# isunLt/U2MKD

Hardware: AMD Instinct MI355X
Metric: LiDAR points/sec/node fwd+bwd (teacher+student+KD), 1/2/4/8 MI355X (higher is better)
Workload: dtype f32 (fp32 products emulated on the 16-bit matrix pipe: f16x2 forward / input gradient, bf16x3 weight gradient; fp32 accumulate)

## Files before the change

include/u2mkd_hip.h:

```cpp
#ifndef U2MKD_HIP_H
#define U2MKD_HIP_H

#include <stddef.h>
#include <stdint.h>

#ifdef __cplusplus
extern "C" {
#endif

typedef void *u2mkd_stream_t;

int u2mkd_version(void);
const char *u2mkd_last_error(void);
int u2mkd_stream_wait_stream(u2mkd_stream_t waiter, u2mkd_stream_t signaler);
void *u2mkd_mailbox_alloc(size_t bytes);
int u2mkd_mailbox_free(void *p);
int u2mkd_mailbox_post(const void *const *srcs, uint32_t is64, int32_t n, int64_t *slot, int64_t seq, u2mkd_stream_t s);

int u2mkd_hash(const int32_t *coords , int64_t n, int64_t *out , u2mkd_stream_t s);
int u2mkd_kernel_hash(const int32_t *coords , const int32_t *offsets , int64_t n,
                      int32_t k, int64_t *out , u2mkd_stream_t s);

size_t u2mkd_hash_table_bytes(int64_t n_refs);
int u2mkd_hash_table_build(const int64_t *refs, int64_t n_refs, void *table, u2mkd_stream_t s);
// ... 358 lines not shown
                                          const int32_t *sort_idx, const int32_t *wstart, const int32_t *wlen,
                                          const int32_t *qc, const float *radial, const float *tq, const float *tk,
                                          const float *tv, int32_t L, int32_t qgl, float split_a, int32_t qc_span,
                                          int64_t n, int32_t h, int32_t hdim, float *delta ,
                                          void *workspace, size_t workspace_bytes, float *dq, float *dk, float *dv,
                                          int64_t ld_grad, float *dtq, float *dtk, float *dtv, u2mkd_stream_t s);
#include "u2mkd_hip_sptr_rows16.h"

int u2mkd_sptr_table_reduce(const void *workspace, int64_t n, int32_t h, int32_t L, float split_a, float *dtq, float *dtk,
                            float *dtv, u2mkd_stream_t s);

int u2mkd_sptr_quant_coords_shifted(const float *xyz , const int32_t *sort_idx , int64_t n, const float *lo,
                                    float wx, float wy, float wz, float shx, float shy, float shz, float qx, float qy,
                                    float qz, int32_t *qc , float *radial , u2mkd_stream_t s);

int u2mkd_sptr_plain_forward_strided(const float *q, const float *k, const float *v, int64_t ld_qkv, float q_scale,
                                     const int32_t *sort_idx, const int32_t *wstart, const int32_t *wlen, int64_t n,
                                     int32_t h, int32_t hdim, float *out, int64_t ld_out, float *lse, u2mkd_stream_t s);
int u2mkd_sptr_plain_backward_strided(const float *q, const float *k, const float *v, int64_t ld_qkv, float q_scale,
                                      const float *out, const float *dout, int64_t ld_out, const float *lse,
                                      const int32_t *sort_idx, const int32_t *wstart, const int32_t *wlen, int64_t n,
                                      int32_t h, int32_t hdim, float *delta , float *dq, float *dk,
                                      float *dv, int64_t ld_grad, u2mkd_stream_t s);

int u2mkd_sptr_precompute_all(int32_t N, int32_t n, uint32_t n_max, const int32_t *counts, const int32_t *offsets,
                              const int32_t *sq_offsets, int32_t *index_0_offsets, int32_t *index_1_offsets,
                              int32_t *index_0, int32_t *index_1, u2mkd_stream_t s);
int u2mkd_sptr_attention_step1_forward(int32_t N_q, int32_t N_k, int32_t M, int32_t h, int32_t hdim, uint32_t n_max,
                                       const float *q, const float *k, const int32_t *index0, const int32_t *index1,
                                       float *attn, u2mkd_stream_t s);
int u2mkd_sptr_attention_step1_backward(int32_t N, int32_t M, int32_t h, int32_t hdim, uint32_t n_max,
                                        const float *grad_out, const int32_t *index0, const int32_t *index0_offsets,
                                        const int32_t *index1, const int32_t *index1_offsets, const float *q,
                                        const float *k, float *grad_q, float *grad_k, u2mkd_stream_t s);
int u2mkd_sptr_attention_step2_forward(int32_t N, int32_t M, int32_t h, int32_t hdim, int32_t n_max, const float *attn,
                                       const float *v, const int32_t *index0_offsets, const int32_t *index1,
                                       float *output, u2mkd_stream_t s);
int u2mkd_sptr_attention_step2_backward(int32_t N, int32_t M, int32_t h, int32_t hdim, int32_t n_max,
                                        const float *grad_out, const int32_t *index0, const int32_t *index0_offsets,
                                        const int32_t *index1, const int32_t *index1_offsets, const float *attn,
                                        const float *v, float *grad_attn, float *grad_v, u2mkd_stream_t s);
int u2mkd_sptr_dot_prod_with_idx_forward(int32_t N, int32_t M, int32_t h, int32_t hdim, int32_t n_max, int32_t L,
                                         const float *q, const int32_t *index_q, const int32_t *index_q_offsets,
                                         const float *k, const int32_t *index_k, const float *table_q,
                                         const float *table_k, const int32_t *rel_idx, float *output,
                                         u2mkd_stream_t s);
int u2mkd_sptr_dot_prod_with_idx_all_forward(int32_t N, int32_t M, int32_t h, int32_t hdim, int32_t n_max, int32_t L,
                                             const float *q, const int32_t *index_q, const int32_t *index_q_offsets,
                                             const float *k, const int32_t *index_k, const float *table_q,
                                             const float *table_k, const int32_t *rel_idx, float *output,
                                             u2mkd_stream_t s);
int u2mkd_sptr_dot_prod_with_idx_backward(int32_t N, int32_t M, int32_t h, int32_t hdim, int32_t n_max, int32_t L,
                                          const float *grad_out, const float *q, const int32_t *index_q_offsets,
                                          const float *k, const int32_t *index_k_offsets, const int32_t *index_k,
                                          const float *table_q, const float *table_k, const int32_t *rel_idx,
                                          float *grad_q, float *grad_k, float *grad_table_q, float *grad_table_k,
                                          u2mkd_stream_t s);
int u2mkd_sptr_attention_step2_with_rel_pos_value_forward(int32_t N, int32_t M, int32_t h, int32_t hdim, int32_t n_max,
                                                          const float *attn, const float *v,
                                                          const int32_t *index0_offsets, const int32_t *index1,
                                                          const float *table, const int32_t *rel_idx, float *output,
                                                          u2mkd_stream_t s);
int u2mkd_sptr_attention_step2_with_rel_pos_value_backward(int32_t N, int32_t M, int32_t h, int32_t hdim, int32_t L,
                                                           int32_t n_max, const float *grad_out, const int32_t *index0,
                                                           const int32_t *index0_offsets, const int32_t *index1,
                                                           const int32_t *index1_offsets, const float *attn,
                                                           const float *v, const float *table, const int32_t *rel_idx,
                                                           float *grad_attn, float *grad_v, float *grad_table,
                                                           u2mkd_stream_t s);

size_t u2mkd_bn2d_workspace_bytes(int64_t b, int32_t c, int64_t hw);
int u2mkd_bn2d_train_forward(const float *x, const float *res, int64_t b, int32_t c, int64_t hw, const float *gamma,
                             const float *beta, float eps, float momentum, int32_t relu, float *running_mean,
                             float *running_var, int64_t *num_batches_tracked, void *workspace,
                             float *mean , float *invstd , float *y, u2mkd_stream_t s);
int u2mkd_bn2d_eval_forward(const float *x, const float *res, int64_t b, int32_t c, int64_t hw, const float *gamma,
                            const float *beta, float eps, int32_t relu, const float *running_mean,
                            const float *running_var, float *y, u2mkd_stream_t s);
int u2mkd_bn2d_backward(const float *dy, const float *x, const float *res, int64_t b, int32_t c, int64_t hw,
                        const float *mean, const float *invstd, const float *gamma, const float *beta, int32_t relu,
                        int32_t batch_stats, void *workspace, float *dgamma, float *dbeta, float *dx,
                        float *dres , u2mkd_stream_t s);

int u2mkd_bn2d_local_stats(const float *x, int64_t b, int32_t c, int64_t hw, void *workspace, float *stats ,
                           u2mkd_stream_t s);
int u2mkd_bn2d_apply(const float *x, const float *res, int64_t b, int32_t c, int64_t hw, const float *mean,
                     const float *invstd, const float *gamma, const float *beta, int32_t relu, float *y, u2mkd_stream_t s);
int u2mkd_bn2d_backward_local(const float *dy, const float *x, const float *res, int64_t b, int32_t c, int64_t hw,
                              const float *mean, const float *invstd, const float *gamma, const float *beta, int32_t relu,
                              void *workspace, float *sums , float *keep ,
                              u2mkd_stream_t s);
int u2mkd_bn2d_backward_apply(const float *dy, const float *x, const float *res, int64_t b, int32_t c, int64_t hw,
                              const float *total_n , const float *mean, const float *invstd, const float *gamma,
                              const float *beta, int32_t relu, const float *sums , float *dx,
                              float *dres , u2mkd_stream_t s);

size_t u2mkd_sptr_tiles_workspace_bytes(int64_t n, int32_t h);
int u2mkd_sptr_attention_forward_tiles(const float *q, const float *k, const float *v, int64_t ld_qkv, float q_scale,
                                       const int32_t *sort_idx, const int32_t *wstart, const int32_t *wlen, const int32_t *qc,
                                       const float *radial, const float *tq, const float *tk, const float *tv, int32_t L,
                                       int32_t qgl, float split_a, int64_t n, int32_t h, int32_t hdim, float *out, int64_t ld_out,
                                       float *lse, void *workspace, size_t workspace_bytes, u2mkd_stream_t s);

int32_t u2mkd_sgd_chunk_elements(void);
int u2mkd_sgd_batch(const int64_t *jobs, int32_t n_jobs, int64_t total_chunks, float lr, float momentum, float weight_decay,
                    int32_t nesterov, int32_t contract, u2mkd_stream_t s);
int u2mkd_grads_unscale_check(const int64_t *jobs, int32_t n_jobs, int64_t total_chunks, const float *inv_scale, float *found_inf,
                              u2mkd_stream_t s);
int u2mkd_sgd_batch_amp(const int64_t *jobs, int32_t n_jobs, int64_t total_chunks, float lr, float momentum, float weight_decay,
                        int32_t nesterov, int32_t contract, const float *grad_scale, const float *found_inf, u2mkd_stream_t s);
int u2mkd_adam_batch(const int64_t *jobs, int32_t n_jobs, int64_t total_chunks, const float *scalars, float decay, float weight_decay,
                     int32_t decoupled, float w1, float beta2, float w2, float eps, int32_t form, u2mkd_stream_t s);
int u2mkd_adam_batch_amp(const int64_t *jobs, int32_t n_jobs, int64_t total_chunks, const float *scalars, int32_t window, float decay,
                         float weight_decay, int32_t decoupled, float w1, float beta2, float w2, float eps, int32_t form,
                         const int32_t *count_in, int32_t *count_out, int32_t count_known, const float *grad_scale,
                         const float *found_inf, u2mkd_stream_t s);
int u2mkd_debug_adam_stage(int32_t stage, int32_t form, const float *a, const float *b, const float *c, float scalar, float *out,
                           int64_t n, u2mkd_stream_t s);

size_t u2mkd_prep_scan_workspace_bytes(int64_t n);
int32_t u2mkd_prep_key_bits(int32_t axis);
int u2mkd_prep_sweep_compact(const float *sweep, int64_t m, void *workspace, int32_t *pos, u2mkd_stream_t s);
int u2mkd_prep_points(const float *key, const int64_t *labels, int64_t nk, const float *sweep, int64_t m, const void *workspace,
                      const int32_t *pos, const int32_t *kseg, const int32_t *mseg, const int32_t *sseg, int32_t n_sweeps,
                      const double *tm, int32_t nb, const double *par, const int32_t *flip, int32_t train, int32_t f32mode,
                      double voxel_size, int64_t ignore_label, float *feats, int32_t *vox, int64_t *labels_full, uint8_t *kf,
                      int32_t *mn, int32_t *off, u2mkd_stream_t s);
int u2mkd_prep_project(const float *key, int64_t nk, const int32_t *kseg, int32_t nb, int32_t ncam, const double *cam, float *pc,
                       uint8_t *masks, uint8_t *pt_with_img, u2mkd_stream_t s);
int u2mkd_prep_voxel_keys(const int32_t *vox, const int32_t *mn, const int32_t *off, int32_t nb, int64_t cap, int64_t *keys,
                          int32_t *err, u2mkd_stream_t s);
int u2mkd_prep_voxel_sets(const int64_t *skeys, const int64_t *perm, int64_t cap, void *workspace, int32_t *rank,
                          const int32_t *off, int32_t nb, const float *feats, const int32_t *vox, const int32_t *mn,
                          const int64_t *labels, const uint8_t *kf, const uint8_t *pt_with_img, const uint8_t *masks,
                          const float *pc, int32_t ncam, int64_t nk, int64_t *inverse_map, int64_t *inds, float *feats_o,
                          int32_t *coords_o, int64_t *labels_o, uint8_t *kf_o, uint8_t *fov_o, uint8_t *masks_o, float *pc_o,
                          int32_t *voxoff, u2mkd_stream_t s);

#ifdef __cplusplus
}
#endif
#endif
```

u2mkd_amd/_lib.py:

```python
from __future__ import annotations

import ctypes as C
import os

import torch

_HERE = os.path.dirname(os.path.abspath(__file__))
LIB_PATH = os.path.join(_HERE, 'lib', 'libu2mkd_hip%s.so' % os.environ.get('U2MKD_LIB_SUFFIX', ''))

_i32, _i64, _sz, _f32, _p = C.c_int32, C.c_int64, C.c_size_t, C.c_float, C.c_void_p

SIGNATURES = {
    'u2mkd_version': (C.c_int, []),
    'u2mkd_last_error': (C.c_char_p, []),
    'u2mkd_hash': (C.c_int, [_p, _i64, _p, _p]),
    'u2mkd_kernel_hash': (C.c_int, [_p, _p, _i64, _i32, _p, _p]),
    'u2mkd_hash_table_bytes': (_sz, [_i64]),
    'u2mkd_hash_table_build': (C.c_int, [_p, _i64, _p, _p]),
    'u2mkd_hash_table_query': (C.c_int, [_p, _i64, _p, _i64, _p, _p]),
    'u2mkd_hash_table_query2': (C.c_int, [_p, _i64, _p, _i64, _p, _p, _p]),
    'u2mkd_kmap_build_table': (C.c_int, [_p, _i64, _p, _i64, _p, _i32, _p, _p]),
    'u2mkd_kmap_invert': (C.c_int, [_p, _i64, _i32, _i64, _p, _p]),
    'u2mkd_kmap_sizes': (C.c_int, [_p, _i64, _i32, _p, _p, _p]),
    'u2mkd_kmap_compact': (C.c_int, [_p, _i64, _i32, _p, _p, _p, _p]),
    'u2mkd_downsample_keys': (C.c_int, [_p, _i64, _i32, _i32, _i32, _p, _p]),
    'u2mkd_downsample_keys_checked': (C.c_int, [_p, _i64, _i32, _i32, _i32, _p, _p, _p]),
    'u2mkd_downsample_keys_general': (C.c_int, [_p, _i64] + [_i32] * 9 + [_p, _i32, _p, _p, _p]),
    'u2mkd_floor_coords': (C.c_int, [_p, _i64, _i32, _p, _p]),
    'u2mkd_unpack_keys': (C.c_int, [_p, _i64, _p, _p]),
    'u2mkd_transpose_weights': (C.c_int, [_p, _i32, _i32, _i32, _p, _p]),
    'u2mkd_conv_forward': (C.c_int, [_p, _i64, _i32, _p, _i32, _p, _i64, _i32, _i32, _p, _p]),
    'u2mkd_conv_forward_sorted': (C.c_int, [_p, _i64, _i32, _p, _i32, _p, _p, _p, _i64, _i32, _i32, _p, _p]),
    'u2mkd_debug_conv_forward_sorted': (C.c_int, [_p, _i64, _i32, _p, _i32, _p, _p, _p, _i64, _i32, _i32, _i32, _p, _p]),
    'u2mkd_conv_lk_supported': (_i32, [_i32, _i32, _i32]),
    'u2mkd_conv_forward_lk': (C.c_int, [_p, _i64, _i32, _p, _i32, _p, _i64, _i64, _i32, _i32, _p, _p]),
    'u2mkd_stream_wait_stream': (C.c_int, [_p, _p]),
    'u2mkd_sgd_chunk_elements': (_i32, []),
    'u2mkd_sgd_batch': (C.c_int, [_p, _i32, _i64, _f32, _f32, _f32, _i32, _i32, _p]),
    'u2mkd_grads_unscale_check': (C.c_int, [_p, _i32, _i64, _p, _p, _p]),
    'u2mkd_sgd_batch_amp': (C.c_int, [_p, _i32, _i64, _f32, _f32, _f32, _i32, _i32, _p, _p, _p]),
    'u2mkd_adam_batch': (C.c_int, [_p, _i32, _i64, _p, _f32, _f32, _i32, _f32, _f32, _f32, _f32, _i32, _p]),
    'u2mkd_adam_batch_amp': (C.c_int, [_p, _i32, _i64, _p, _i32, _f32, _f32, _i32, _f32, _f32, _f32, _f32, _i32, _p, _p, _i32, _p, _p, _p]),
    'u2mkd_debug_adam_stage': (C.c_int, [_i32, _i32, _p, _p, _p, _f32, _p, _i64, _p]),
    'u2mkd_mailbox_alloc': (_p, [_sz]),
    'u2mkd_mailbox_free': (C.c_int, [_p]),
    'u2mkd_mailbox_post': (C.c_int, [_p, C.c_uint32, _i32, _p, _i64, _p]),
    'u2mkd_conv_tiles_supported': (_i32, [_i32, _i32, _i32]),
    'u2mkd_conv_tiles_arith': (_i32, [_i32, _i32, _i32]),
    'u2mkd_weight_fragments_bytes': (_sz, [_i32, _i32, _i32, _i32]),
    'u2mkd_weight_fragments': (C.c_int, [_p, _i32, _i32, _i32, _i32, _i32, _p, _p]),
    'u2mkd_weight_fragments_batch': (C.c_int, [_p, _i32, _i64, _p]),
    'u2mkd_conv_forward_tiles': (C.c_int, [_p, _i64, _i32, _p, _i32, _p, _p, _p, _p, _i64, _i32, _i32, _i32, _p, _p]),
    'u2mkd_conv_forward_tiles_ep': (C.c_int, [_p, _i64, _i32, _p, _i32, _p, _p, _p, _p, _i64, _i32, _i32, _i32, _p, _p, _p, _i32, _p, _p]),
    'u2mkd_pairs_gather_sum_ep': (C.c_int, [_p, _p, _i64, _i32, _i32, _p, _p, _p, _i32, _p, _p]),
    'u2mkd_pairs_gather_sum_stats_slab_rows': (_i32, []),
    'u2mkd_pairs_gather_sum_stats_supported': (_i32, [_i32]),
    'u2mkd_pairs_gather_sum_stats': (C.c_int, [_p, _p, _i64, _i32, _i32, _p, _p, _p]),
    'u2mkd_debug_conv_tile_pairs_stamps': (C.c_int, [_p, _i64, _p, _p, _p, _p, _p, _i64, _i32, _i32, _p, _p, _p]),
    'u2mkd_debug_wgrad_stamps': (C.c_int, [_p, _p, _p, _p, _i64, _i32, _p, _p, _p]),
    'u2mkd_conv_forward_pairs': (C.c_int, [_p, _i64, _i32, _p, _i32, _p, _p, _p, _i64, _i32, _i32, _p, _p]),
    'u2mkd_conv_pairs_x3_supported': (_i32, [_i32, _i32]),
    'u2mkd_conv_forward_pairs_x3': (C.c_int, [_p, _i64, _i32, _p, _i32, _p, _p, _p, _i64, _i32, _p, _p]),
    'u2mkd_linear_forward': (C.c_int, [_p, _i64, _i32, _p, _i32, _p, _i32, _p, _p]),
    'u2mkd_bn2d_workspace_bytes': (C.c_size_t, [_i64, _i32, _i64]),
    'u2mkd_bn2d_train_forward': (C.c_int, [_p, _p, _i64, _i32, _i64, _p, _p, C.c_float, C.c_float, _i32, _p, _p, _p, _p, _p, _p, _p, _p]),
    'u2mkd_bn2d_eval_forward': (C.c_int, [_p, _p, _i64, _i32, _i64, _p, _p, C.c_float, _i32, _p, _p, _p, _p]),
    'u2mkd_bn2d_backward': (C.c_int, [_p, _p, _p, _i64, _i32, _i64, _p, _p, _p, _p, _i32, _i32, _p, _p, _p, _p, _p, _p]),
    'u2mkd_bn2d_local_stats': (C.c_int, [_p, _i64, _i32, _i64, _p, _p, _p]),
    'u2mkd_bn2d_apply': (C.c_int, [_p, _p, _i64, _i32, _i64, _p, _p, _p, _p, _i32, _p, _p]),
    'u2mkd_bn2d_backward_local': (C.c_int, [_p, _p, _p, _i64, _i32, _i64, _p, _p, _p, _p, _i32, _p, _p, _p, _p]),
    'u2mkd_bn2d_backward_apply': (C.c_int, [_p, _p, _p, _i64, _i32, _i64, _p, _p, _p, _p, _p, _i32, _p, _p, _p, _p]),
    'u2mkd_linear_forward_x3': (C.c_int, [_p, _i64, _i32, _p, _i32, _p, _p, _p]),
    'u2mkd_conv_pairs_f16x2_supported': (_i32, [_i32, _i32]),
    'u2mkd_conv_forward_pairs_f16x2': (C.c_int, [_p, _i64, _i32, _p, _i32, _p, _p, _p, _i64, _i32, _p, _p]),
    'u2mkd_linear_forward_f16x2': (C.c_int, [_p, _i64, _i32, _p, _i32, _p, _p, _p]),
    'u2mkd_pairs_capacity': (_i64, [_i64, _i64, _i32]),
    'u2mkd_pairs_build': (C.c_int, [_p, _i64, _i64, _i32, _p, _p, _p, _p, _p, _p, _p, _p, _p]),
    'u2mkd_pairs_gather_sum': (C.c_int, [_p, _p, _i64, _i32, _i32, _p, _p]),
    'u2mkd_kmap_rowmask': (C.c_int, [_p, _i64, _i32, _p, _p]),
    'u2mkd_tile_schedule_workspace_bytes': (_sz, [_i64]),
    'u2mkd_tile_schedule': (C.c_int, [_p, _p, _i64, _i32, _i32, _i32, _p, _p, _p, _p, _p]),
    'u2mkd_wgrad_plan_ints': (_i32, [_i32]),
    'u2mkd_wgrad_plan': (C.c_int, [_p, _i32, _i64, _p, _p]),
    'u2mkd_conv_wgrad_pairs_workspace_bytes': (_sz, [_i64, _i32, _i32, _i32]),
    'u2mkd_conv_wgrad_pairs': (C.c_int, [_p, _i32, _p, _i32, _p, _p, _i64, _i32, _i32, _p, _sz, _p, _p]),
    'u2mkd_conv_forward_tiles_bf16': (C.c_int, [_p, _i64, _i32, _p, _i32, _p, _p, _p, _p, _i64, _i32, _i32, _p, _p]),
    'u2mkd_conv_forward_tiles_f16': (C.c_int, [_p, _i64, _i32, _p, _i32, _p, _p, _p, _p, _i64, _i32, _i32, _p, _p]),
    'u2mkd_conv_wgrad_pairs_bf16': (C.c_int, [_p, _i32, _p, _i32, _p, _p, _i64, _i32, _i32, _p, _sz, _p, _p]),
    'u2mkd_conv_wgrad_pairs_f16': (C.c_int, [_p, _i32, _p, _i32, _p, _p, _i64, _i32, _i32, _p, _sz, _p, _p]),
    'u2mkd_conv_forward_pairs_bf16': (C.c_int, [_p, _i64, _i32, _p, _i32, _p, _p, _p, _i64, _i32, _p, _p]),
    'u2mkd_conv_forward_pairs_f16': (C.c_int, [_p, _i64, _i32, _p, _i32, _p, _p, _p, _i64, _i32, _p, _p]),
    'u2mkd_linear_forward_bf16': (C.c_int, [_p, _i64, _i32, _p, _i32, _p, _p, _p]),
    'u2mkd_linear_forward_f16': (C.c_int, [_p, _i64, _i32, _p, _i32, _p, _p, _p]),
    'u2mkd_pairs_gather_sum_bf16': (C.c_int, [_p, _p, _i64, _i32, _i32, _p, _p]),
    'u2mkd_pairs_gather_sum_f16': (C.c_int, [_p, _p, _i64, _i32, _i32, _p, _p]),
    'u2mkd_convolution_workspace_bytes': (_sz, [_i64, _i64, _i32, _i32, _p, _i32]),
    'u2mkd_convolution_forward': (C.c_int, [_p, _i64, _i32, _p, _i64, _i32, _p, _p, _p, _i32, _i32, _p, _sz, _p]),
    'u2mkd_convolution_backward': (C.c_int, [_p, _i64, _i32, _p, _p, _i64, _i32, _p, _p, _p, _p, _i32, _i32, _p, _sz, _p]),
    'u2mkd_bn_num_slabs': (_i64, [_i64]),
    'u2mkd_bn_train_forward': (C.c_int, [_p, _p, _i32, _i64, _i32, _p, _p, _f32, _f32, _p, _p, _p, _i32, _p, _p, _p, _p, _p]),
    'u2mkd_bn_train_forward_from_partial': (C.c_int, [_p, _p, _i64, _i32, _p, _p, _f32, _f32, _p, _p, _p, _i32, _p, _i32, _p, _p, _p, _p]),
    'u2mkd_bn_eval_forward': (C.c_int, [_p, _p, _i32, _i64, _i32, _p, _p, _f32, _p, _p, _i32, _p, _p, _p]),
    'u2mkd_bn_backward': (C.c_int, [_p, _p, _p, _i32, _i64, _i32, _p, _p, _p, _p, _i32, _i32, _p, _p, _p, _p, _p, _p]),
    'u2mkd_bn_local_stats': (C.c_int, [_p, _i32, _i64, _i32, _p, _p, _p]),
    'u2mkd_bn_merge_stats': (C.c_int, [_p, _i32, _i32, _f32, _f32, _p, _p, _p, _p, _p, _p, _p]),
    'u2mkd_bn_apply': (C.c_int, [_p, _p, _i32, _i64, _i32, _p, _p, _p, _p, _i32, _p, _p]),
    'u2mkd_bn_backward_local': (C.c_int, [_p, _p, _p, _i32, _i64, _i32, _p, _p, _p, _p, _i32, _p, _p, _p, _p]),
    'u2mkd_bn_backward_apply': (C.c_int, [_p, _p, _p, _i32, _i64, _i32, _p, _p, _p, _p, _p, _i32, _p, _p, _p, _p]),
    'u2mkd_ln_num_slabs': (_i64, [_i64, _i32]),
    'u2mkd_ln_forward': (C.c_int, [_p, _i32, _i64, _i32, _p, _p, _f32, _p, _p, _p, _p]),
    'u2mkd_ln_add_forward': (C.c_int, [_p, _p, _p, _i32, _i64, _i32, _p, _p, _f32, _p, _p, _p, _p, _p]),
    'u2mkd_ln_backward': (C.c_int, [_p, _p, _p, _p, _i32, _i64, _i32, _p, _p, _p, _p, _p, _p, _p, _p, _p]),
    'u2mkd_scene_num_slabs': (_i64, [_i64, _i64]),
    'u2mkd_scene_slabs': (C.c_int, [_p, _i64, _i64, _p, _p, _i64, _p]),
    'u2mkd_gn_forward': (C.c_int, [_p, _i32, _i64, _i32, _i32, _p, _p, _p, _p, _p, _i64, _i64, _p, _p, _f32, _p, _p, _p, _p, _p]),
    'u2mkd_gn_backward': (C.c_int, [_p, _p, _i32, _i64, _i32, _i32, _p, _p, _p, _p, _p, _i64, _i64, _p, _p, _p, _p, _p, _p, _p, _p, _p]),
    'u2mkd_scene_pool_forward': (C.c_int, [_p, _i32, _i64, _i32, _i32, _p, _p, _p, _p, _i64, _i64, _p, _p, _p, _p]),
    'u2mkd_scene_pool_backward': (C.c_int, [_p, _i32, _i64, _i32, _i32, _p, _p, _p, _i64, _p, _p]),
    'u2mkd_bev_plan': (C.c_int, [_p, _i64] + [_i32] * 12 + [_p, _p, _p, _p]),
    'u2mkd_bev_tables': (C.c_int, [_p, _p, _i64, _i64, _i32, _p, _p, _p]),
    'u2mkd_bev_segment_mean': (C.c_int, [_p, _i32, _i64, _i32, _p, _p, _i64, _p, _p]),
    'u2mkd_bev_dense_store': (C.c_int, [_p, _i32, _i64, _i32, _p, _p, _i64, _i32, _i32, _i32, _p, _p]),
    'u2mkd_bev_dense_gather': (C.c_int, [_p, _i32, _i64, _i32, _p, _p, _i64, _i32, _i32, _i32, _p, _p]),
    'u2mkd_sptr_window_keys': (C.c_int, [_p, _p, _i64, _p, _p, _f32, _f32, _f32, _p, _p]),
    'u2mkd_select_mse_partials': (_i32, []),
    'u2mkd_select_mse_forward': (C.c_int, [_p, _p, _p, _i64, _i32, _p, _p, _p, _p]),
    'u2mkd_select_mse_backward': (C.c_int, [_p, _p, _p, _p, _p, _p, _i64, _i32, _p, _p, _p]),
    'u2mkd_sptr_plan_prepare_workspace_bytes': (_sz, []),
    'u2mkd_sptr_plan_prepare': (C.c_int, [_p, _p, _i64, _f32, _f32, _f32, _f32, _f32, _f32, _p, _p, _p, _p, _p, _p]),
    'u2mkd_sptr_window_ranges': (C.c_int, [_p, _i64, _p, _p, _p]),
    'u2mkd_sptr_quant_coords': (C.c_int, [_p, _p, _i64, _p, _f32, _f32, _f32, _f32, _f32, _f32, _p, _p, _p]),
    'u2mkd_sptr_attention_forward': (C.c_int, [_p, _p, _p, _p, _p, _p, _p, _p, _p, _p, _p, _i32, _i32, _f32, _i64, _i32, _i32, _p, _p, _p]),
    'u2mkd_sptr_backward_workspace_bytes': (_sz, [_i64, _i32, _i32]),
    'u2mkd_sptr_attention_backward': (C.c_int, [_p] * 14 + [_i32, _i32, _f32, _i32, _i64, _i32, _i32] + [_p, _p, _sz] + [_p] * 7),
    'u2mkd_sptr_tiles_workspace_bytes': (_sz, [_i64, _i32]),
    'u2mkd_sptr_attention_forward_tiles': (C.c_int, [_p, _p, _p, _i64, _f32] + [_p] * 8 + [_i32, _i32, _f32, _i64, _i32, _i32, _p, _i64, _p, _p, _sz, _p]),
    'u2mkd_sptr_attention_forward_strided': (C.c_int, [_p, _p, _p, _i64, _f32] + [_p] * 8 + [_i32, _i32, _f32, _i64, _i32, _i32, _p, _i64, _p, _p]),
    'u2mkd_sptr_attention_backward_strided': (C.c_int, [_p, _p, _p, _i64, _f32, _p, _p, _i64] + [_p] * 9 + [_i32, _i32, _f32, _i32, _i64, _i32, _i32]
                                              + [_p, _p, _sz] + [_p, _p, _p, _i64, _p, _p, _p, _p]),
    'u2mkd_sptr_table_reduce': (C.c_int, [_p, _i64, _i32, _i32, _f32, _p, _p, _p, _p]),
    'u2mkd_sptr_quant_coords_shifted': (C.c_int, [_p, _p, _i64, _p] + [_f32] * 9 + [_p, _p, _p]),
    'u2mkd_sptr_plain_forward_strided': (C.c_int, [_p, _p, _p, _i64, _f32, _p, _p, _p, _i64, _i32, _i32, _p, _i64, _p, _p]),
    'u2mkd_sptr_plain_backward_strided': (C.c_int, [_p, _p, _p, _i64, _f32, _p, _p, _i64, _p, _p, _p, _p, _i64, _i32, _i32,
                                                    _p, _p, _p, _p, _i64, _p]),
    'u2mkd_sptr_precompute_all': (C.c_int, [_i32, _i32, C.c_uint32] + [_p] * 8),
    'u2mkd_sptr_attention_step1_forward': (C.c_int, [_i32, _i32, _i32, _i32, _i32, C.c_uint32] + [_p] * 6),
    'u2mkd_sptr_attention_step1_backward': (C.c_int, [_i32, _i32, _i32, _i32, C.c_uint32] + [_p] * 10),
    'u2mkd_sptr_attention_step2_forward': (C.c_int, [_i32] * 5 + [_p] * 6),
    'u2mkd_sptr_attention_step2_backward': (C.c_int, [_i32] * 5 + [_p] * 10),
    'u2mkd_sptr_dot_prod_with_idx_forward': (C.c_int, [_i32] * 6 + [_p] * 10),
    'u2mkd_sptr_dot_prod_with_idx_all_forward': (C.c_int, [_i32] * 6 + [_p] * 10),
    'u2mkd_sptr_dot_prod_with_idx_backward': (C.c_int, [_i32] * 6 + [_p] * 14),
    'u2mkd_sptr_attention_step2_with_rel_pos_value_forward': (C.c_int, [_i32] * 5 + [_p] * 8),
    'u2mkd_sptr_attention_step2_with_rel_pos_value_backward': (C.c_int, [_i32] * 6 + [_p] * 13),
# ... 110 lines not shown
```

u2mkd_amd/camera.py:

```python
import os

import torch
import torch.nn.functional as F
from torch import nn

__all__ = ['SwiftNetRes18', 'SwiftNetResNet', 'BNReluConv', 'BatchNorm2d', 'SyncBatchNorm2d', 'bn_act']

_HIP_BN2D = os.environ.get('U2MKD_BN2D', '1') != '0'


class _MaxPool3s2Function(torch.autograd.Function):
    @staticmethod
    def forward(ctx, x):
        from . import _lib as L
        n, c, h, w = x.shape
        oh, ow = (h - 1) // 2 + 1, (w - 1) // 2 + 1
        y = torch.empty(n, c, oh, ow, dtype=torch.float32, device=x.device)
        code = torch.empty(n, c, oh, ow, dtype=torch.uint8, device=x.device)
        L.call('u2mkd_maxpool3s2_forward', L.ptr(x), n * c, h, w, L.ptr(y), L.ptr(code), L.stream())
        ctx.save_for_backward(code)
        ctx.shape = (n, c, h, w)
        return y

    @staticmethod
# ... 173 lines not shown
        hw = h * w
        dev, st = x.device, L.stream()
        ws = torch.empty(max(L.load().u2mkd_bn2d_workspace_bytes(b, c, hw), 16), dtype=torch.uint8, device=dev)
        stats = torch.empty(2 * c + 1, dtype=torch.float32, device=dev)
        L.call('u2mkd_bn2d_local_stats', L.ptr(x), b, c, hw, L.ptr(ws), L.ptr(stats), st)
        note_collective('all_gather', stats)
        if world > 1:
            gathered = torch.empty(world, 2 * c + 1, dtype=torch.float32, device=dev)
            _gather_rows(gathered, stats, group)
        else:
            gathered = stats.view(1, -1)
        mit = torch.empty(2 * c + 1, dtype=torch.float32, device=dev)
        mean, invstd, total = mit[:c], mit[c:2 * c], mit[2 * c:]
        track = bn.running_mean is not None
        L.call('u2mkd_bn_merge_stats', L.ptr(gathered), world, c, float(bn.eps), float(bn.momentum if track else 0.0),
               L.ptr(bn.running_mean if track else None), L.ptr(bn.running_var if track else None), L.ptr(mean),
               L.ptr(invstd), L.ptr(total), L.ptr(bn.num_batches_tracked if track else None), L.stream())
        if track:
            torch._C._increment_version([t for t in (bn.running_mean, bn.running_var, bn.num_batches_tracked) if t is not None])
        y = torch.empty_like(x)
        L.call('u2mkd_bn2d_apply', L.ptr(x), L.ptr(res), b, c, hw, L.ptr(mean), L.ptr(invstd), L.ptr(weight), L.ptr(bias),
               int(relu), L.ptr(y), L.stream())
        ctx.save_for_backward(x, weight, bias, res, mean, invstd, total)
        ctx.relu, ctx.group, ctx.world = bool(relu), group, world
        return y

    @staticmethod
    def backward(ctx, dy):
        from . import _lib as L
        from .torchsparse.nn.functional import _sum_over_ranks, note_collective
        x, weight, bias, res, mean, invstd, total = ctx.saved_tensors
        b, c, h, w = x.shape
        hw = h * w
        dy = dy.contiguous()
        dev = x.device
        ws = torch.empty(max(L.load().u2mkd_bn2d_workspace_bytes(b, c, hw), 16), dtype=torch.uint8, device=dev)
        both = torch.empty(2, 2 * c, dtype=torch.float32, device=dev)
        sums, local = both[0], both[1]
        L.call('u2mkd_bn2d_backward_local', L.ptr(dy), L.ptr(x), L.ptr(res), b, c, hw, L.ptr(mean), L.ptr(invstd),
               L.ptr(weight), L.ptr(bias), int(ctx.relu), L.ptr(ws), L.ptr(sums), L.ptr(local), L.stream())
        note_collective('all_reduce', sums)
        if ctx.world > 1:
            _sum_over_ranks(sums, ctx.group)
        dx = torch.empty_like(x)
        dres = torch.empty_like(x) if res is not None else None
        L.call('u2mkd_bn2d_backward_apply', L.ptr(dy), L.ptr(x), L.ptr(res), b, c, hw, L.ptr(total), L.ptr(mean),
               L.ptr(invstd), L.ptr(weight), L.ptr(bias), int(ctx.relu), L.ptr(sums), L.ptr(dx), L.ptr(dres), L.stream())
        return (dx, local[c:] if weight is not None else None, local[:c] if bias is not None else None, dres,
                None, None, None, None)


class SyncBatchNorm2d(nn.SyncBatchNorm):

    def forward(self, x, relu=False, residual=None):
        from .torchsparse.nn.functional import _sync_group
        sync = _sync_group(self) if self.training else None
        if (sync is not None and _HIP_BN2D and x.is_cuda and x.dtype == torch.float32 and x.dim() == 4 and x.is_contiguous()
                and x.numel() > 0 and not torch.is_autocast_enabled() and self.momentum is not None
                and (residual is None or (residual.dtype == x.dtype and residual.shape == x.shape))):
            if residual is not None:
                residual = residual.contiguous()
            return _SyncBatchNorm2dFunction.apply(x, self.weight, self.bias, residual, self, relu, sync[0], sync[1])
        if (sync is None and _HIP_BN2D and x.is_cuda and x.dtype == torch.float32 and x.dim() == 4 and x.is_contiguous()
                and x.numel() > 0 and not torch.is_autocast_enabled() and (self.momentum is not None or not self.training)
                and (residual is None or (residual.dtype == x.dtype and residual.shape == x.shape))):
            if residual is not None:
                residual = residual.contiguous()
            return _BatchNorm2dFunction.apply(x, self.weight, self.bias, residual, self, relu)
        y = super().forward(x)
        if residual is not None:
            y = y + residual
        return F.relu(y) if relu else y


def bn_act(bn, x, relu=False, residual=None):
    if isinstance(bn, (BatchNorm2d, SyncBatchNorm2d)):
        return bn(x, relu, residual)
    y = bn(x)
    if residual is not None:
        y = y + residual
    return F.relu(y) if relu else y


class _Conv2dFunction(torch.autograd.Function):

    @staticmethod
    def forward(ctx, x, weight, stride, padding):
        ctx.dtypes = (x.dtype, weight.dtype)
        ctx.pid = id(weight)
        if torch.is_autocast_enabled('cuda'):
            dt = torch.get_autocast_dtype('cuda')
            x, weight = x.to(dt), weight.to(dt)
        ctx.save_for_backward(x, weight)
        ctx.conf = (stride, padding)
        with torch.autocast('cuda', enabled=False):
            return F.conv2d(x, weight, None, stride, padding)

    @staticmethod
    def backward(ctx, g):
        from . import deferred
        x, weight = ctx.saved_tensors
        stride, padding = ctx.conf
        g = g.contiguous().to(x.dtype)

        def bwd(mask):
            return torch.ops.aten.convolution_backward(g, x, weight, None, stride, padding, (1, 1), False, (0, 0), 1, mask)
        gx = bwd((True, False, False))[0].to(ctx.dtypes[0]) if ctx.needs_input_grad[0] else None
        gw = None
        if ctx.needs_input_grad[1]:
            if deferred.owned(ctx.pid):
                deferred.join()
                gw = bwd((False, True, False))[1].to(ctx.dtypes[1])
            else:
                side = deferred.side_for('camera_wgrad', g.device, owner=ctx.pid)
                with torch.cuda.stream(side):
                    gw = bwd((False, True, False))[1].to(ctx.dtypes[1])
                for t in (x, weight, g):
                    t.record_stream(side)
                gw.record_stream(torch.cuda.current_stream(g.device))
        return gx, gw, None, None


class Conv2d(nn.Conv2d):

    def forward(self, x):
        from . import deferred
        w = self.weight
        if (deferred.enabled() and deferred.overlap_ok() and x.is_cuda and torch.is_grad_enabled() and w.requires_grad and w.is_leaf and w.grad is None and self.bias is None
                and self.groups == 1 and self.dilation == (1, 1) and self.padding_mode == 'zeros'
                and not isinstance(self.padding, str) and not torch.cuda.is_current_stream_capturing()):
            return _Conv2dFunction.apply(x, w, self.stride, self.padding)
        return super().forward(x)


class BasicBlock(nn.Module):
    expansion = 1

    def __init__(self, inplanes, planes, stride=1, downsample=None):
        super().__init__()
        self.conv1 = Conv2d(inplanes, planes, 3, stride, 1, bias=False)
        self.bn1 = BatchNorm2d(planes)
        self.relu = nn.ReLU(inplace=True)
        self.conv2 = Conv2d(planes, planes, 3, 1, 1, bias=False)
        self.bn2 = BatchNorm2d(planes)
        self.downsample = downsample

    def forward(self, x):
        out = bn_act(self.bn1, self.conv1(x), relu=True)
        out = bn_act(self.bn2, self.conv2(out), relu=True, residual=x if self.downsample is None else self.downsample(x))
        return out, out


class BNReluConv(nn.Sequential):
    def __init__(self, cin, cout, k=3, bn_momentum=0.1):
        super().__init__()
        self.add_module('norm', BatchNorm2d(cin, momentum=bn_momentum))
        self.add_module('relu', nn.ReLU(inplace=True))
        self.add_module('conv', Conv2d(cin, cout, kernel_size=k, padding=k // 2, bias=False))

    def forward(self, x):
        return self.conv(bn_act(self.norm, x, relu=True))


class SpatialPyramidPooling(nn.Module):
    def __init__(self, cin, num_levels, bt_size, level_size, out_size, grids, bn_momentum):
        super().__init__()
        self.grids = grids
        self.spp = nn.Sequential()
        self.spp.add_module('spp_bn', BNReluConv(cin, bt_size, k=1, bn_momentum=bn_momentum))
        final = bt_size
        for i in range(num_levels):
            final += level_size
            self.spp.add_module('spp' + str(i), BNReluConv(bt_size, level_size, k=1, bn_momentum=bn_momentum))
        self.spp.add_module('spp_fuse', BNReluConv(final, out_size, k=1, bn_momentum=bn_momentum))

    def forward(self, x):
        h, w = x.shape[2:4]
        ar = w / h
        x = self.spp[0](x)
        levels = [x]
        for i in range(1, len(self.spp) - 1):
            grid = (self.grids[i - 1], max(1, round(ar * self.grids[i - 1])))
            levels.append(_up(self.spp[i](F.adaptive_avg_pool2d(x, grid)), (h, w)))
        return self.spp[-1](torch.cat(levels, 1))


class _Upsample(nn.Module):
    def __init__(self, cin, cskip, cout, k=3):
        super().__init__()
        self.bottleneck = BNReluConv(cskip, cin, k=1)
        self.blend_conv = BNReluConv(cin, cout, k=k)

    def forward(self, x, skip):
        skip = self.bottleneck(skip)
        return self.blend_conv(_up(x, skip.shape[2:4], skip))


class SwiftNetResNet(nn.Module):
    def __init__(self, layers=(2, 2, 2, 2), num_features=(128, 128, 128), spp_grids=(8, 4, 2, 1)):
# ... 77 lines not shown
```

Baseline: 1.230 million.

## Add native bf16x3 MFMA weight-gradient kernel for camera 3x3 convs

Adds a HIP kernel that computes the 3x3 stride-1 conv weight gradient directly, replacing aten convolution_backward for supported shapes (channels multiples of 64, up to 128x128). Inputs are split into three bf16 planes and multiplied on the matrix pipe with LDS-staged rows and register-shifted taps. Work is split across blocks into per-block partial slabs, which a second kernel then reduces. The aim is to make the camera-branch wgrad cheaper than the vendor path, at the cost of extra workspace and a separate reduction pass.

```diff
diff --git a/include/u2mkd_hip.h b/include/u2mkd_hip.h
--- a/include/u2mkd_hip.h
+++ b/include/u2mkd_hip.h
@@ -464,6 +464,11 @@
                         int32_t batch_stats, void *workspace, float *dgamma, float *dbeta, float *dx,
                         float *dres , u2mkd_stream_t s);
 
+int u2mkd_conv2d_wgrad3x3_supported(int32_t cin, int32_t cout, int32_t h, int32_t w);
+size_t u2mkd_conv2d_wgrad3x3_workspace_bytes(int64_t n, int32_t cin, int32_t cout, int32_t h, int32_t w);
+int u2mkd_conv2d_wgrad3x3(const float *x, const float *dy, int64_t n, int32_t cin, int32_t cout, int32_t h, int32_t w,
+                          void *workspace, size_t workspace_bytes, float *dw, u2mkd_stream_t s);
+
 int u2mkd_bn2d_local_stats(const float *x, int64_t b, int32_t c, int64_t hw, void *workspace, float *stats ,
                            u2mkd_stream_t s);
 int u2mkd_bn2d_apply(const float *x, const float *res, int64_t b, int32_t c, int64_t hw, const float *mean,
diff --git a/u2mkd_amd/_lib.py b/u2mkd_amd/_lib.py
--- a/u2mkd_amd/_lib.py
+++ b/u2mkd_amd/_lib.py
@@ -70,6 +70,9 @@
     'u2mkd_bn2d_apply': (C.c_int, [_p, _p, _i64, _i32, _i64, _p, _p, _p, _p, _i32, _p, _p]),
     'u2mkd_bn2d_backward_local': (C.c_int, [_p, _p, _p, _i64, _i32, _i64, _p, _p, _p, _p, _i32, _p, _p, _p, _p]),
     'u2mkd_bn2d_backward_apply': (C.c_int, [_p, _p, _p, _i64, _i32, _i64, _p, _p, _p, _p, _p, _i32, _p, _p, _p, _p]),
+    'u2mkd_conv2d_wgrad3x3_supported': (_i32, [_i32, _i32, _i32, _i32]),
+    'u2mkd_conv2d_wgrad3x3_workspace_bytes': (_sz, [_i64, _i32, _i32, _i32, _i32]),
+    'u2mkd_conv2d_wgrad3x3': (C.c_int, [_p, _p, _i64, _i32, _i32, _i32, _i32, _p, _sz, _p, _p]),
     'u2mkd_linear_forward_x3': (C.c_int, [_p, _i64, _i32, _p, _i32, _p, _p, _p]),
     'u2mkd_conv_pairs_f16x2_supported': (_i32, [_i32, _i32]),
     'u2mkd_conv_forward_pairs_f16x2': (C.c_int, [_p, _i64, _i32, _p, _i32, _p, _p, _p, _i64, _i32, _p, _p]),
diff --git a/u2mkd_amd/camera.py b/u2mkd_amd/camera.py
--- a/u2mkd_amd/camera.py
+++ b/u2mkd_amd/camera.py
@@ -279,6 +279,27 @@
     return F.relu(y) if relu else y
 
 
+_NATIVE_WGRAD = os.environ.get('U2MKD_CAMERA_WGRAD', '1') != '0'
+
+
+def _weight_grad(g, x, weight, stride, padding, bwd):
+    from torch.nn.modules.utils import _pair
+    if (_NATIVE_WGRAD and x.is_cuda and x.dtype == g.dtype == weight.dtype == torch.float32 and x.dim() == 4 and x.numel() > 0
+            and x.is_contiguous() and g.is_contiguous() and tuple(weight.shape[2:]) == (3, 3) and _pair(stride) == (1, 1)
+            and _pair(padding) == (1, 1) and g.shape[2:] == x.shape[2:]):
+        from . import _lib as L
+        lib = L.load()
+        n, cin, h, w = x.shape
+        cout = weight.shape[0]
+        if lib.u2mkd_conv2d_wgrad3x3_supported(cin, cout, h, w):
+            nbytes = lib.u2mkd_conv2d_wgrad3x3_workspace_bytes(n, cin, cout, h, w)
+            ws = torch.empty(nbytes, dtype=torch.uint8, device=x.device)
+            gw = torch.empty(weight.shape, dtype=torch.float32, device=x.device)
+            L.call('u2mkd_conv2d_wgrad3x3', L.ptr(x), L.ptr(g), n, cin, cout, h, w, L.ptr(ws), nbytes, L.ptr(gw), L.stream())
+            return gw
+    return bwd((False, True, False))[1]
+
+
 class _Conv2dFunction(torch.autograd.Function):
 
     @staticmethod
@@ -302,16 +323,19 @@
 
         def bwd(mask):
             return torch.ops.aten.convolution_backward(g, x, weight, None, stride, padding, (1, 1), False, (0, 0), 1, mask)
+
+        def wgrad():
+            return _weight_grad(g, x, weight, stride, padding, bwd)
         gx = bwd((True, False, False))[0].to(ctx.dtypes[0]) if ctx.needs_input_grad[0] else None
         gw = None
         if ctx.needs_input_grad[1]:
             if deferred.owned(ctx.pid):
                 deferred.join()
-                gw = bwd((False, True, False))[1].to(ctx.dtypes[1])
+                gw = wgrad().to(ctx.dtypes[1])
             else:
                 side = deferred.side_for('camera_wgrad', g.device, owner=ctx.pid)
                 with torch.cuda.stream(side):
-                    gw = bwd((False, True, False))[1].to(ctx.dtypes[1])
+                    gw = wgrad().to(ctx.dtypes[1])
                 for t in (x, weight, g):
                     t.record_stream(side)
                 gw.record_stream(torch.cuda.current_stream(g.device))
diff --git a/u2mkd_amd/csrc/conv2d_wgrad.hip b/u2mkd_amd/csrc/conv2d_wgrad.hip
--- /dev/null
+++ b/u2mkd_amd/csrc/conv2d_wgrad.hip
@@ -0,0 +1,257 @@
+#include "conv_internal.h"
+
+namespace u2mkd {
+
+namespace {
+
+constexpr int kCwChunk = 32;
+constexpr int kCwRowElems = 40;
+constexpr int kCwRowBytes = 2 * kCwRowElems;
+constexpr int kCwPlane = 64 * kCwRowBytes;
+constexpr int kCwSlot = 3 * kCwPlane;
+constexpr int kCwGroups = 10;
+constexpr int kCwStage = (64 * kCwGroups + 255) / 256;
+constexpr int kCwTargetWgs = 512;
+constexpr size_t kCwMaxWorkspace = (size_t)96 << 20;
+
+typedef short cw_s16x4 __attribute__((ext_vector_type(4)));
+
+struct CwPlanes { uint2 p[3]; };
+__device__ __forceinline__ CwPlanes cw_split4(const f32x4 &v) {
+    uint32_t h[4], m[4], l[4];
+#pragma unroll
+    for (int i = 0; i < 4; ++i) {
+        h[i] = __float_as_uint(v[i]) & 0xffff0000u;
+        const float r1 = v[i] - __uint_as_float(h[i]);
+        m[i] = __float_as_uint(r1) & 0xffff0000u;
+        const float r2 = r1 - __uint_as_float(m[i]);
+        l[i] = __float_as_uint(r2);
+    }
+    CwPlanes p;
+    p.p[0] = make_uint2(__builtin_amdgcn_perm(h[1], h[0], 0x07060302u), __builtin_amdgcn_perm(h[3], h[2], 0x07060302u));
+    p.p[1] = make_uint2(__builtin_amdgcn_perm(m[1], m[0], 0x07060302u), __builtin_amdgcn_perm(m[3], m[2], 0x07060302u));
+    p.p[2] = make_uint2(__builtin_amdgcn_perm(l[1], l[0], 0x07060302u), __builtin_amdgcn_perm(l[3], l[2], 0x07060302u));
+    return p;
+}
+
+__device__ __forceinline__ f32x4 cw_mfma(const uint2 &a, const uint2 &b, f32x4 c) {
+    return __builtin_amdgcn_mfma_f32_16x16x16bf16_1k(__builtin_bit_cast(cw_s16x4, a), __builtin_bit_cast(cw_s16x4, b), c, 0, 0, 0);
+}
+
+__device__ __forceinline__ int cw_slot(int q) { return (q + 3) % 3; }
+
+__global__ void __launch_bounds__(256) __attribute__((amdgpu_waves_per_eu(2, 2)))
+conv2d_wgrad3x3_kernel(const float *__restrict__ x, const float *__restrict__ dy, int cin, int cout, int h, int w, int nrows,
+                       int chunks, float *__restrict__ slabs) {
+    __shared__ __attribute__((aligned(16))) char smem[3 * kCwSlot];
+    const int tid = threadIdx.x, lane = tid & 63, wave = tid >> 6;
+    const int gq = lane >> 4, li = lane & 15;
+    const int wy = wave >> 1, wx = wave & 1;
+    const int tiles_ci = cin / 64;
+    const int co0 = (blockIdx.y / tiles_ci) * 64, ci0 = (blockIdx.y % tiles_ci) * 64;
+    const int64_t items = (int64_t)chunks * nrows;
+    const int t0 = (int)(items * blockIdx.x / gridDim.x), t1 = (int)(items * (blockIdx.x + 1) / gridDim.x);
+
+    f32x4 acc[2][2][3][3];
+#pragma unroll
+    for (int m = 0; m < 2; ++m)
+#pragma unroll
+        for (int n = 0; n < 2; ++n)
+#pragma unroll
+            for (int ky = 0; ky < 3; ++ky)
+#pragma unroll
+                for (int kx = 0; kx < 3; ++kx) acc[m][n][ky][kx] = (f32x4){0.f, 0.f, 0.f, 0.f};
+
+    auto stage_load = [&](int q, int c0, f32x4 (&v)[kCwStage]) __attribute__((always_inline)) {
+        const bool row_ok = q >= 0 && q < nrows;
+        const int img = row_ok ? q / h : 0, y = row_ok ? q - img * h : 0;
+#pragma unroll
+        for (int i = 0; i < kCwStage; ++i) {
+            const int g = tid + 256 * i;
+            const int ch = g / kCwGroups, xg = c0 - 4 + 4 * (g - ch * kCwGroups);
+            v[i] = (f32x4){0.f, 0.f, 0.f, 0.f};
+            if (row_ok && g < 64 * kCwGroups && xg >= 0 && xg < w)
+                v[i] = *reinterpret_cast<const f32x4 *>(x + (((size_t)img * cin + ci0 + ch) * h + y) * (size_t)w + xg);
+        }
+    };
+    auto stage_store = [&](int q, const f32x4 (&v)[kCwStage]) __attribute__((always_inline)) {
+        char *slot = smem + cw_slot(q) * kCwSlot;
+#pragma unroll
+        for (int i = 0; i < kCwStage; ++i) {
+            const int g = tid + 256 * i;
+            if (g >= 64 * kCwGroups) continue;
+            const int ch = g / kCwGroups, j = g - ch * kCwGroups;
+            const CwPlanes p = cw_split4(v[i]);
+            char *d = slot + ch * kCwRowBytes + 8 * j - 4;
+#pragma unroll
+            for (int pl = 0; pl < 3; ++pl) {
+                if (j > 0) *reinterpret_cast<uint32_t *>(d + pl * kCwPlane) = p.p[pl].x;
+                *reinterpret_cast<uint32_t *>(d + pl * kCwPlane + 4) = p.p[pl].y;
+            }
+        }
+    };
+    auto load_dy = [&](int cc, int r, int ks, f32x4 (&v)[2]) __attribute__((always_inline)) {
+        const int img = r / h, y = r - img * h;
+        const int xk = cc * kCwChunk + 16 * ks + 4 * gq;
+#pragma unroll
+        for (int m = 0; m < 2; ++m) {
+            v[m] = (f32x4){0.f, 0.f, 0.f, 0.f};
+            if (xk < w)
+                v[m] = *reinterpret_cast<const f32x4 *>(dy + (((size_t)img * cout + co0 + 32 * wy + 16 * m + li) * h + y) * (size_t)w + xk);
+        }
+    };
+
+    if (t0 < t1) {
+        f32x4 dy_next[2], pre[kCwStage];
+        load_dy(t0 / nrows, t0 % nrows, 0, dy_next);
+        for (int t = t0; t < t1; ++t) {
+            const int cc = t / nrows, r = t - cc * nrows;
+            const int c0 = cc * kCwChunk;
+            const int img = r / h, y = r - img * h;
+            const int nks = min(2, (w - c0 + 15) / 16);
+            if (t == t0 || r == 0) {
+                __syncthreads();
+                for (int q = r - 1; q <= r + 1; ++q) {
+                    stage_load(q, c0, pre);
+                    stage_store(q, pre);
+                }
+                __syncthreads();
+            }
+            const bool more = t + 1 < t1 && r + 1 < nrows;
+            if (more) stage_load(r + 2, c0, pre);
+            for (int ks = 0; ks < nks; ++ks) {
+                CwPlanes a[2];
+#pragma unroll
+                for (int m = 0; m < 2; ++m) a[m] = cw_split4(dy_next[m]);
+                if (ks + 1 < nks) load_dy(cc, r, ks + 1, dy_next);
+                else if (t + 1 < t1) load_dy((t + 1) / nrows, (t + 1) % nrows, 0, dy_next);
+#pragma unroll
+                for (int ky = 0; ky < 3; ++ky) {
+                    const int yy = y + ky - 1;
+                    if (yy < 0 || yy >= h) continue;
+                    const char *slot = smem + cw_slot(r + ky - 1) * kCwSlot + (32 * wx + li) * kCwRowBytes + (16 * ks + 4 * gq) * 2;
+#pragma unroll
+                    for (int n = 0; n < 2; ++n) {
+                        uint2 b[3][3];
+#pragma unroll
+                        for (int pl = 0; pl < 3; ++pl) {
+                            const char *src = slot + pl * kCwPlane + 16 * n * kCwRowBytes;
+                            const uint2 lo = *reinterpret_cast<const uint2 *>(src), hi = *reinterpret_cast<const uint2 *>(src + 8);
+                            b[pl][0] = make_uint2(__builtin_amdgcn_alignbit(lo.y, lo.x, 16), __builtin_amdgcn_alignbit(hi.x, lo.y, 16));
+                            b[pl][1] = make_uint2(lo.y, hi.x);
+                            b[pl][2] = make_uint2(__builtin_amdgcn_alignbit(hi.x, lo.y, 16), __builtin_amdgcn_alignbit(hi.y, hi.x, 16));
+                        }
+                        constexpr int PA[6] = {2, 0, 1, 1, 0, 0}, PB[6] = {0, 2, 1, 0, 1, 0};
+#pragma unroll
+                        for (int p = 0; p < 6; ++p)
+#pragma unroll
+                            for (int m = 0; m < 2; ++m)
+#pragma unroll
+                                for (int kx = 0; kx < 3; ++kx)
+                                    acc[m][n][ky][kx] = cw_mfma(a[m].p[PA[p]], b[PB[p]][kx], acc[m][n][ky][kx]);
+                    }
+                }
+            }
+            if (more) {
+                __syncthreads();
+                stage_store(r + 2, pre);
+                __syncthreads();
+            }
+        }
+    }
+    float *slab = slabs + (size_t)blockIdx.x * cout * cin * 9;
+#pragma unroll
+    for (int m = 0; m < 2; ++m)
+#pragma unroll
+        for (int reg = 0; reg < 4; ++reg)
+#pragma unroll
+            for (int n = 0; n < 2; ++n) {
+                const int co = co0 + 32 * wy + 16 * m + 4 * gq + reg, ci = ci0 + 32 * wx + 16 * n + li;
+                float *d = slab + ((size_t)co * cin + ci) * 9;
+#pragma unroll
+                for (int ky = 0; ky < 3; ++ky)
+#pragma unroll
+                    for (int kx = 0; kx < 3; ++kx) d[3 * ky + kx] = acc[m][n][ky][kx][reg];
+            }
+}
+
+__global__ void __launch_bounds__(256)
+conv2d_wgrad3x3_reduce_kernel(const float *__restrict__ slabs, int nslab, int64_t elems, float *__restrict__ dw) {
+    __shared__ float4 part[16][16];
+    const int lx = threadIdx.x & 15, g = threadIdx.x >> 4;
+    const int64_t e = ((int64_t)blockIdx.x * 16 + lx) * 4;
+    float4 acc = make_float4(0.f, 0.f, 0.f, 0.f);
+    if (e < elems) {
+        for (int j = g; j < nslab; j += 64) {
+            float4 v[4];
+#pragma unroll
+            for (int i = 0; i < 4; ++i) {
+                const int jj = j + 16 * i;
+                v[i] = jj < nslab ? *reinterpret_cast<const float4 *>(slabs + (size_t)jj * elems + e) : make_float4(0.f, 0.f, 0.f, 0.f);
+            }
+#pragma unroll
+            for (int i = 0; i < 4; ++i) { acc.x += v[i].x; acc.y += v[i].y; acc.z += v[i].z; acc.w += v[i].w; }
+        }
+    }
+    part[g][lx] = acc;
+    __syncthreads();
+    if (g == 0 && e < elems) {
+        float4 t = part[0][lx];
+#pragma unroll
+        for (int i = 1; i < 16; ++i) {
+            const float4 v = part[i][lx];
+            t.x += v.x; t.y += v.y; t.z += v.z; t.w += v.w;
+        }
+        *reinterpret_cast<float4 *>(dw + e) = t;
+    }
+}
+
+bool cw_shape_ok(int64_t n, int cin, int cout, int h, int w) {
+    return n > 0 && h > 0 && w > 0 && cin > 0 && cout > 0 && cin % 64 == 0 && cout % 64 == 0 && w % 4 == 0 && cin <= 4096 &&
+           cout <= 4096 && n * h * ceil_div(w, kCwChunk) < ((int64_t)1 << 30);
+}
+
+int cw_splits(int64_t n, int cin, int cout, int h, int w) {
+    const int64_t items = n * h * ceil_div(w, kCwChunk), tiles = (int64_t)(cin / 64) * (cout / 64);
+    const int64_t slab = (int64_t)cin * cout * 9 * sizeof(float);
+    int64_t s = kCwTargetWgs / tiles;
+    if (s > (int64_t)(kCwMaxWorkspace / slab)) s = (int64_t)(kCwMaxWorkspace / slab);
+    if (s > items) s = items;
+    return (int)(s < 1 ? 1 : s);
+}
+
+}
+
+}
+
+using namespace u2mkd;
+
+extern "C" {
+
+int u2mkd_conv2d_wgrad3x3_supported(int32_t cin, int32_t cout, int32_t h, int32_t w) {
+    return cw_shape_ok(1, cin, cout, h, w) && (int64_t)cin * cout <= 128 * 128 ? 1 : 0;
+}
+
+size_t u2mkd_conv2d_wgrad3x3_workspace_bytes(int64_t n, int32_t cin, int32_t cout, int32_t h, int32_t w) {
+    if (!cw_shape_ok(n, cin, cout, h, w)) return 0;
+    return (size_t)cw_splits(n, cin, cout, h, w) * cin * cout * 9 * sizeof(float);
+}
+
+int u2mkd_conv2d_wgrad3x3(const float *x, const float *dy, int64_t n, int32_t cin, int32_t cout, int32_t h, int32_t w,
+                          void *workspace, size_t workspace_bytes, float *dw, u2mkd_stream_t s) {
+    U2_REQUIRE(x && dy && workspace && dw, "u2mkd_conv2d_wgrad3x3: null pointer");
+    U2_REQUIRE(cw_shape_ok(n, cin, cout, h, w), "u2mkd_conv2d_wgrad3x3: shape n %lld, %d -> %d channels, %d x %d not supported",
+               (long long)n, cin, cout, h, w);
+    U2_REQUIRE(workspace_bytes >= u2mkd_conv2d_wgrad3x3_workspace_bytes(n, cin, cout, h, w),
+               "u2mkd_conv2d_wgrad3x3: workspace of %zu bytes is too small", workspace_bytes);
+    const int splits = cw_splits(n, cin, cout, h, w);
+    const int64_t elems = (int64_t)cin * cout * 9;
+    float *slabs = reinterpret_cast<float *>(workspace);
+    hipLaunchKernelGGL(conv2d_wgrad3x3_kernel, dim3((unsigned)splits, (unsigned)((cin / 64) * (cout / 64))), dim3(256), 0, as_stream(s),
+                       x, dy, cin, cout, h, w, (int)(n * h), (int)ceil_div(w, kCwChunk), slabs);
+    hipLaunchKernelGGL(conv2d_wgrad3x3_reduce_kernel, dim3((unsigned)ceil_div(elems, 64)), dim3(256), 0, as_stream(s), slabs, splits,
+                       elems, dw);
+    return check_launch("u2mkd_conv2d_wgrad3x3");
+}
+
+}
```

Result: slower. 1.204 million (-2.1%).
